# scalable-arch/CAL_22-MPC

Measured on AMD Instinct MI355X. Metric: 64B blocks/s (whole node) + achieved HBM GB/s fraction; ratio bit-exact vs CPU, higher is better.
Workload: dtype u8; 1 GPU; 268435456 random_u32 64 B blocks per GPU, VPC probe config (6 modules, all predictors); algorithm=VPC, line_size=64, blocks_per_gpu=268435456

## Files before the change

cal_22-mpc_amd/csrc/mpc_vpc_lane.hip:

```cpp
#include "mpc_kernel_common.h"
#include "mpc_ring.h"

#ifndef MPC_JIT_BM
#define MPC_JIT_BM 0
#endif
#ifndef MPC_JIT_ANYROOT
#define MPC_JIT_ANYROOT 0
#endif
#ifndef MPC_JIT_PLANES
#define MPC_JIT_PLANES 0
#endif
#ifndef MPC_JIT_GATHER
#define MPC_JIT_GATHER 0
#endif
#ifndef MPC_JIT_WSHIFT
#define MPC_JIT_WSHIFT 0
#endif
#ifndef MPC_ABLATE
#define MPC_ABLATE 0
#endif
namespace {

constexpr int LK_PW = 8;
constexpr int LK_PW2 = 16;
__device__ __host__ constexpr int lk_base(int kind) { return kind & 7; }
__device__ __host__ constexpr int lk_dist(int kind) { return (kind & LK_PW2) ? 2 : ((kind & LK_PW) ? 1 : 0); }

typedef const u32 __attribute__((address_space(4))) *ctab_t;
__device__ __forceinline__ ctab_t lane_tab(const MpcVpcParams &P) { return (ctab_t)(u64)P.tab; }

#if MPC_JIT_ANYROOT || MPC_JIT_GATHER || MPC_JIT_WSHIFT
template <int Q>
__device__ __forceinline__ MpcFastModule lane_fm_const(const MpcVpcParams &P)
{
  MpcFastModule f = P.fm[Q];
#if MPC_JIT_ANYROOT
  constexpr int roots[] = {MPC_JIT_ROOTS};
  f.root = roots[Q];
#endif
#if MPC_JIT_GATHER
  constexpr int gathers[] = {MPC_JIT_GATHERS};
  f.gather = gathers[Q] ? Q + 1 : 0;
#endif
#if MPC_JIT_WSHIFT
  constexpr int wgens[] = {MPC_JIT_WGENS};
  f.wgen = wgens[Q] ? Q + 1 : 0;
#endif
  return f;
}
#define LANE_FM(Q) lane_fm_const<Q>(P)
#else
#define LANE_FM(Q) P.fm[Q]
#endif

template <int W>
struct Lane {
  u32 x[W];
  u32 b0;
  u32 rootb;
  bool gen;
  ctab_t trunc;
};

template <int W>
__device__ __forceinline__ u32 lane_root_bytes(const Lane<W> &c, int root)
{
  const int rw = root >> 2;
  u32 xw = 0;
#pragma unroll
  for (int e = 0; e < (MPC_JIT_ANYROOT ? W : 4); e++) xw = and_or(c.x[e], 0u - (u32)(e == rw), xw);
  return perm(xw, xw, 0x01010101u * (u32)(root & 3));
}
__device__ __forceinline__ u32 lane_onebase_pred(u32 rb, int root, int e)
{
  const u32 here = (e == (root >> 2)) ? (0xffu << (8 * (root & 3))) : 0u;
  return rb & ~here;
}
__device__ __forceinline__ u32 lane_row0_word(u32 msbs, int root, int e)
{
  return (MPC_JIT_ANYROOT && e == 3 && root > 15) ? (msbs & 0x00ffffffu) : msbs;
}
template <int W, int NR>
__device__ __forceinline__ void lane_root_to_front(const Lane<W> &c, int root, u32 (&r)[W])
{
  u32 prev = lane_root_bytes<W>(c, root) & 0xff000000u;
#pragma unroll
  for (int e = 0; e < (MPC_JIT_ANYROOT ? NR : (NR < 4 ? NR : 4)); e++) {
    const u32 sh = alignbyte(r[e], prev, 3);
    const int nb = root + 1 - 4 * e;
    const u32 m = nb >= 4 ? ~0u : (nb <= 0 ? 0u : ((1u << (8 * nb)) - 1u));
    prev = r[e];
    r[e] = mask_sel(m, sh, r[e]);
  }
}

__device__ __forceinline__ u32 msb_of_bsub(u32 a, u32 b) { return ((a | H80) - (b & L7F)) ^ a ^ ~b; }

template <int W>
__device__ __forceinline__ u32 plane_bytes(const u32 (&x)[W], int q, int k)
{
  const u32 s01 = k >= 2 ? 0x07030602u : 0x05010400u;
  const u32 p01 = perm(x[4 * q + 1], x[4 * q], s01), p23 = perm(x[4 * q + 3], x[4 * q + 2], s01);
  return perm(p23, p01, (k & 1) ? 0x07060302u : 0x05040100u);
}

template <int W>
__device__ __forceinline__ u32 shuffled_word(const u32 (&x)[W], int j)
{
  constexpr int NG = W / 4;
  return plane_bytes<W>(x, j % NG, 3 - j / NG);
}

template <int KIND>
__device__ __forceinline__ u32 window_predict(u32 b, u32 c1, u32 c2, const MpcFastModule &fm)
{
  if constexpr (KIND == MPC_FK_DIFF)
    return ((b & L7F) + c1) ^ ((b & H80) ^ c2);
  else if constexpr (KIND == MPC_FK_WEIGHT)
    return (b & c1) | ((b >> fm.rs2) & c2);
  else
    return (((b << fm.ls1) >> fm.rs1) & c1) | (((b << fm.ls2) >> fm.rs2) & c2);
}

#if MPC_JIT_GATHER
template <int W>
__device__ __forceinline__ u32 lane_gather_base(const Lane<W> &c, int q, int e)
{
  constexpr short bases[][4 * W] = {MPC_JIT_BASES};
  u32 half[2];
#pragma unroll
  for (int h = 0; h < 2; h++) {
    const int b0 = bases[q][4 * e + 2 * h], b1 = bases[q][4 * e + 2 * h + 1];
    const u32 w0 = b0 >= 0 ? c.x[b0 >> 2] : 0u, w1 = b1 >= 0 ? c.x[b1 >> 2] : 0u;
    const u32 sel = (b0 >= 0 ? (u32)(b0 & 3) : 0x0cu) | ((b1 >= 0 ? 4u + (u32)(b1 & 3) : 0x0cu) << 8) | 0x0c0c0000u;
    half[h] = perm(w1, w0, sel);
  }
  return perm(half[1], half[0], 0x05040100u);
}
#endif

#if MPC_JIT_WSHIFT
template <int W>
__device__ __forceinline__ u32 lane_weight_general(u32 b, int q, int e)
{
  constexpr signed char sh[][4 * W] = {MPC_JIT_SHIFTS};
  u32 pred = 0;
#pragma unroll
  for (int k = 0; k < 4; k++) {
    const int s = sh[q][4 * e + k];
    if (s == 99) continue;
    const u32 keep = (s >= 0 ? ((0xffu << s) & 0xffu) : (0xffu >> -s)) << (8 * k);
    pred |= (s >= 0 ? (b << s) : (b >> -s)) & keep;
  }
  return pred;
}
#endif

template <int W, int KIND>
__device__ __forceinline__ u32 window_base(const Lane<W> &c, int e, ctab_t t)
{
  constexpr int D = lk_dist(KIND);
  if (D && e >= D) return c.x[e - D];
  return perm(c.x[e], e ? c.x[e - 1] : 0u, t[e]);
}

template <int W, int KIND, bool FULL = true>
__device__ __forceinline__ u32 window_residue(const Lane<W> &c, int e, ctab_t t, const MpcFastModule &fm)
{
#if MPC_JIT_GATHER
  const u32 b = fm.gather ? lane_gather_base<W>(c, fm.gather - 1, e) : window_base<W, KIND>(c, e, t);
#else
  const u32 b = window_base<W, KIND>(c, e, t);
#endif
  constexpr int D = lk_dist(KIND);
  const int k = D == 2 ? (e < 2 ? e : 2 + (e & 1)) : (D == 1 ? (e ? 1 : 0) : e);
  if constexpr (lk_base(KIND) == MPC_FK_WEIGHT) {
    const u32 p7 = ((b >> fm.rs2) & t[2 * W + k]) | (b & t[3 * W + k]);
    const u32 sub = (c.x[e] | H80) - p7;
    const u32 w = c.x[e] ^ (b & t[4 * W + k]);
    return FULL ? (sub ^ (~w & H80)) : (sub ^ ~w);
  } else {
#if MPC_JIT_WSHIFT
    const u32 pred = fm.wgen ? lane_weight_general<W>(b, fm.wgen - 1, e) : window_predict<lk_base(KIND)>(b, t[W + k], t[2 * W + k], fm);
#else
    const u32 pred = window_predict<lk_base(KIND)>(b, t[W + k], t[2 * W + k], fm);
#endif
    return FULL ? bsub(c.x[e], pred) : msb_of_bsub(c.x[e], pred);
  }
}

template <int W, int KIND, int NR = W>
__device__ __forceinline__ void lane_residue(const Lane<W> &c, const MpcFastModule &fm, ctab_t tab,
                                             u32 (&r)[W], u32 &root_r)
{
  root_r = 0;
  if constexpr (lk_base(KIND) == MPC_FK_ONEBASE) {
    if (c.gen && fm.root != 0) {
      const u32 rb = lane_root_bytes<W>(c, fm.root);
#pragma unroll
      for (int e = 0; e < NR; e++) r[e] = bsub(c.x[e], (MPC_JIT_ANYROOT || e < 4) ? lane_onebase_pred(rb, fm.root, e) : rb);
    } else {
      r[0] = bsub(c.x[0], c.rootb & 0xffffff00u);
#pragma unroll
      for (int e = 1; e < NR; e++) r[e] = bsub(c.x[e], c.rootb);
    }
  } else if constexpr (lk_base(KIND) == MPC_FK_CONSEC) {
    u32 in[NR];
#pragma unroll
    for (int j = 0; j < NR; j++) in[j] = shuffled_word<W>(c.x, j);
    r[0] = bsub(c.x[0], in[0] << 8);
#pragma unroll
    for (int e = 1; e < NR; e++) r[e] = bsub(c.x[e], alignbyte(in[e], in[e - 1], 3));
    root_r = (c.b0 - (c.x[0] >> 24)) & 0xffu;
  } else {
    ctab_t t = tab + fm.tab_off;
#pragma unroll
    for (int e = 0; e < NR; e++) r[e] = window_residue<W, KIND>(c, e, t, fm);
  }
}

template <int W, int KIND, int E0, int E1>
__device__ __forceinline__ u32 lane_row0(const Lane<W> &c, const MpcFastModule &fm, ctab_t tab)
{
  u32 m = 0;
  if constexpr (lk_base(KIND) == MPC_FK_ONEBASE) {
    if (c.gen && fm.root != 0) {
      const u32 rb = lane_root_bytes<W>(c, fm.root);
#pragma unroll
      for (int e = E0; e < E1; e++) m |= lane_row0_word(msb_of_bsub(c.x[e], lane_onebase_pred(rb, fm.root, e)), fm.root, e);
      if (MPC_JIT_ANYROOT && E0 == 0 && fm.root > 15) m |= rb;
    } else {
#pragma unroll
      for (int e = E0; e < E1; e++) m |= msb_of_bsub(c.x[e], e ? c.rootb : (c.rootb & 0xffffff00u));
    }
  } else if constexpr (lk_base(KIND) == MPC_FK_CONSEC) {
#pragma unroll
    for (int e = E0; e < E1; e++) {
      const u32 in_e = shuffled_word<W>(c.x, e);
      m |= msb_of_bsub(c.x[e], e ? alignbyte(in_e, shuffled_word<W>(c.x, e - 1), 3) : (in_e << 8));
    }
  } else {
    ctab_t t = tab + fm.tab_off;
#pragma unroll
    for (int e = E0; e < E1; e++) m |= lane_row0_word(window_residue<W, KIND, false>(c, e, t, fm), c.gen ? fm.root : 0, e);
    if (MPC_JIT_ANYROOT && c.gen && E0 == 0 && fm.root > 15) m |= lane_root_bytes<W>(c, fm.root);
  }
  return m & H80;
}

template <int W>
__device__ __forceinline__ u32 lane_leading_zero_rows(const u32 (&r)[W], ctab_t scan_mask = nullptr, u32 plane_mask = ~0u)
{
  constexpr int NG = W / 4;
  u32 S[NG], G = 0;
  if (scan_mask) {
#pragma unroll
    for (int j = 0; j < NG; j++) {
      S[j] = (r[4 * j] & scan_mask[4 * j]) | (r[4 * j + 1] & scan_mask[4 * j + 1]) | (r[4 * j + 2] & scan_mask[4 * j + 2]) |
             (r[4 * j + 3] & scan_mask[4 * j + 3]);
      G |= S[j];
    }
  } else {
#pragma unroll
    for (int j = 0; j < NG; j++) {
      S[j] = r[4 * j] | r[4 * j + 1] | r[4 * j + 2] | r[4 * j + 3];
      G |= S[j];
    }
  }
  const u32 gf = fold8(G) & plane_mask;
  const u32 p = (u32)__clz((int)gf) - 24u;
  const u32 B = H80 >> (p & 7u);
  u32 j_star = NG - 1;
#pragma unroll
  for (int j = NG - 2; j >= 0; j--) j_star = (S[j] & B) ? (u32)j : j_star;
  return (plane_mask == ~0u ? G : gf) ? NG * p + j_star : 2u * W;
}

template <int W>
struct LaneBest {
  u32 r[W];
  u32 z;
  int q;
  u32 root_r;
  u32 cx;
  u32 pm;
  u32 encb;
};

#ifndef MPC_DEFER_MAX
#define MPC_DEFER_MAX 8
#endif

#ifndef MPC_PAIR_PROBE
#define MPC_PAIR_PROBE 64
#endif
constexpr u32 kPairProbe = MPC_PAIR_PROBE;

__host__ __device__ static inline size_t lane_stats_smem(int K, int bins)
{
  return 16 * (size_t)((2 * K * 8 + 15) / 16) + 16 * (size_t)(((K * bins + 2) * 4 + 15) / 16);
}

template <int W, int KIND>
__device__ __forceinline__ u32 lane_row0_bm(const Lane<W> &c, const MpcFastModule &fm, ctab_t tab)
{
  u32 r[W], root_r;
  lane_residue<W, KIND, 1>(c, fm, tab, r, root_r);
  return r[0] & (c.trunc ? (c.trunc[0] & 0xffffu) : 0xffffu);
}

template <int W, int NPT, int Q>
__device__ __forceinline__ u32 lane_row0_min(const Lane<W> &, const MpcVpcParams &) { return ~0u; }

template <int W, int NPT, int Q, int KIND, int... REST>
__device__ __forceinline__ u32 lane_row0_min(const Lane<W> &c, const MpcVpcParams &P)
{
  if constexpr (Q + 1 == NPT) {
    return ~0u;
  } else {
    const u32 m = MPC_JIT_BM ? lane_row0_bm<W, KIND>(c, LANE_FM(Q), lane_tab(P)) : lane_row0<W, KIND, 0, 3>(c, LANE_FM(Q), lane_tab(P));
    return min(m, lane_row0_min<W, NPT, Q + 1, REST...>(c, P));
  }
}

template <int W, int NPT, int Q>
__device__ __forceinline__ u32 lane_prefilters(const Lane<W> &, const MpcVpcParams &, u64 &, u64 &, bool, bool &) { return 0; }

template <int W, int NPT, int Q, int KIND, int... REST>
__device__ __forceinline__ u32 lane_prefilters(const Lane<W> &c, const MpcVpcParams &P, u64 &need_mask, u64 &defer_mask,
                                               bool allow_defer, bool &alt)
{
  if constexpr (Q + 1 == NPT) {
    return 0;
  } else {
    u32 bit = 0;
    if constexpr (!(MPC_ABLATE & 8)) {
      u32 msb = MPC_JIT_BM ? lane_row0_bm<W, KIND>(c, LANE_FM(Q), lane_tab(P)) : lane_row0<W, KIND, 0, 3>(c, LANE_FM(Q), lane_tab(P));
      if ((__ballot(msb != 0) & need_mask) != need_mask) {
        if (!MPC_JIT_BM) msb |= lane_row0<W, KIND, 3, 4>(c, LANE_FM(Q), lane_tab(P));
        const u64 pass = ~__ballot(msb != 0) & need_mask;
        if (pass) {
          if (MPC_DEFER_MAX > 0 && W <= 16 && allow_defer && __popcll(pass) <= MPC_DEFER_MAX) {
            defer_mask |= pass;
            need_mask &= ~pass;
          } else {
            bit = 1u << Q;
            const u64 even = 0x5555555555555555ull;
            if (__popcll(pass) >= 16 && ((pass & even) == 0 || (pass & ~even) == 0) &&
                __popcll(need_mask & ~pass) >= 16)
              alt = true;
          }
        }
      }
    }
    return bit | lane_prefilters<W, NPT, Q + 1, REST...>(c, P, need_mask, defer_mask, allow_defer, alt);
  }
}

template <int W, int NR>
__device__ __forceinline__ u32 lane_leading_zero_rows_bm(const u32 (&r)[W], ctab_t scan_mask, u32 none);

template <int W, int NPT, int Q>
__device__ __forceinline__ void lane_seq(const Lane<W> &, const MpcVpcParams &, u32, LaneBest<W> &, bool) {}

template <int W, int NPT, int Q, int KIND, int... REST>
__device__ __forceinline__ void lane_seq(const Lane<W> &c, const MpcVpcParams &P, u32 keep_bits, LaneBest<W> &best,
                                         bool any_full)
{
  constexpr bool last = Q + 1 == NPT;
  if (last || (keep_bits & (1u << Q))) {
    u32 r[W], root_r;
    lane_residue<W, KIND>(c, LANE_FM(Q), lane_tab(P), r, root_r);
    if (c.gen && LANE_FM(Q).root != 0) lane_root_to_front<W, W>(c, LANE_FM(Q).root, r);
    const u32 pm_q = MPC_JIT_PLANES ? LANE_FM(Q).plane_mask : (c.gen ? P.plane_mask : ~0u);
    const u32 z = MPC_JIT_BM ? lane_leading_zero_rows_bm<W, W>(r, c.gen ? c.trunc : nullptr, 2u * W)
                             : lane_leading_zero_rows<W>(r, c.gen ? c.trunc : nullptr, pm_q);
    if (!any_full) {
      best.z = z;
      best.q = Q;
      best.root_r = root_r;
      best.cx = (u32)LANE_FM(Q).cx;
      best.pm = pm_q;
      best.encb = (u32)P.enc_bits[P.start + Q + 1];
#pragma unroll
      for (int e = 0; e < W; e++) best.r[e] = r[e];
    } else {
      const u32 m = best.z <= z ? ~0u : 0u;
      best.z = mask_sel(m, z, best.z);
      best.q = (int)mask_sel(m, (u32)Q, (u32)best.q);
      best.root_r = mask_sel(m, root_r, best.root_r);
      best.cx = mask_sel(m, (u32)LANE_FM(Q).cx, best.cx);
      if (MPC_JIT_PLANES) best.pm = mask_sel(m, pm_q, best.pm);
      best.encb = mask_sel(m, (u32)P.enc_bits[P.start + Q + 1], best.encb);
#pragma unroll
      for (int e = 0; e < W; e++) best.r[e] = mask_sel(m, r[e], best.r[e]);
    }
    any_full = true;
  }
  if constexpr (!last) lane_seq<W, NPT, Q + 1, REST...>(c, P, keep_bits, best, any_full);
}

template <int W, int NPT, int Q>
__device__ __forceinline__ void lane_last(const Lane<W> &, const MpcVpcParams &, LaneBest<W> &) {}

template <int W, int NPT, int Q, int KIND, int... REST>
__device__ __forceinline__ void lane_last(const Lane<W> &c, const MpcVpcParams &P, LaneBest<W> &best)
{
  if constexpr (Q + 1 == NPT) {
    lane_residue<W, KIND>(c, LANE_FM(Q), lane_tab(P), best.r, best.root_r);
    if (c.gen && LANE_FM(Q).root != 0) lane_root_to_front<W, W>(c, LANE_FM(Q).root, best.r);
    best.q = Q;
    best.cx = (u32)LANE_FM(Q).cx;
    best.pm = MPC_JIT_PLANES ? LANE_FM(Q).plane_mask : ~0u;
    best.encb = (u32)P.enc_bits[P.start + Q + 1];
  } else {
    lane_last<W, NPT, Q + 1, REST...>(c, P, best);
  }
}


template <int W, int NR>
__device__ __forceinline__ u32 lane_leading_zero_rows_bm(const u32 (&r)[W], ctab_t scan_mask, u32 none)
{
  u32 fe = NR, fw = 0;
#pragma unroll
  for (int e = NR - 1; e >= 0; e--) {
    const u32 v = scan_mask ? (r[e] & scan_mask[e]) : r[e];
    fe = v ? (u32)e : fe;
    fw = v ? v : fw;
  }
  const u32 byte = 4u * fe + ((u32)__builtin_ctz(fw | 0x80000000u) >> 3);
  return fe == (u32)NR ? none : (byte >> 1);
}

template <int W>
__device__ __forceinline__ u32 lane_encode_bm(const u32 (&t)[W])
{
  u32 bits = 0;
  u64 Z = 0;
#pragma unroll
  for (int e = 0; e < W; e++) {
    const u32 hw = perm(t[e], t[e], 0x02030001u);
#pragma unroll
    for (int k = 0; k < 2; k++) {
      const u32 h = k ? (hw >> 16) : (hw & 0xffffu);
      const u32 ones = (u32)__popc(h);
      const bool adj = (h & (h >> 1)) != 0u;
      const bool half_empty = (h & 0xff00u) == 0u || (h & 0x00ffu) == 0u;
      const u32 cost = ones == 1u ? 7u : (ones == 2u && adj) ? 8u : half_empty ? 12u : 17u;
      bits += h ? cost : 0u;
      Z |= (u64)(h == 0u ? 1u : 0u) << (2 * e + k);
    }
  }
  const u64 all = W == 32 ? ~0ull : ((1ull << (2 * (W & 31))) - 1ull);
  const u64 starts = Z & ~(Z << 1);
  const u64 longer = starts & (Z >> 1) & all;
  return bits + 4u * (u32)__popcll(starts) + 3u * (u32)__popcll(longer);
}

template <int W>
__device__ __forceinline__ u32 lane_word_at(const u32 (&x)[W], int idx)
{
  u32 w = 0;
#pragma unroll
  for (int e = 0; e < W; e++) w = and_or(x[e], 0u - (u32)(e == idx), w);
  return w;
}

template <int W, int NR>
__device__ __forceinline__ void lane_residue_rt(const Lane<W> &c, const MpcVpcParams &P, const MpcFastModule &fm, u32 (&r)[W],
                                                u32 &root_r)
{
  switch (fm.kind) {
  case MPC_FK_ONEBASE:
    if (fm.root == 0) {
      lane_residue<W, MPC_FK_ONEBASE, NR>(c, fm, lane_tab(P), r, root_r);
    } else {
      const int rw = fm.root >> 2, rk = fm.root & 3;
      const u32 xw = lane_word_at<W>(c.x, rw);
      const u32 rb = ((xw >> (8 * rk)) & 0xffu) * 0x01010101u;
      const u32 here = 0xffu << (8 * rk);
#pragma unroll
      for (int e = 0; e < NR; e++) r[e] = bsub(c.x[e], e == rw ? (rb & ~here) : rb);
      root_r = 0;
    }
    break;
  case MPC_FK_CONSEC: lane_residue<W, MPC_FK_CONSEC, NR>(c, fm, lane_tab(P), r, root_r); break;
  case MPC_FK_DIFF:
    if (fm.prev_word == 2) lane_residue<W, MPC_FK_DIFF | LK_PW2, NR>(c, fm, lane_tab(P), r, root_r);
    else if (fm.prev_word == 1) lane_residue<W, MPC_FK_DIFF | LK_PW, NR>(c, fm, lane_tab(P), r, root_r);
    else lane_residue<W, MPC_FK_DIFF, NR>(c, fm, lane_tab(P), r, root_r);
    break;
  case MPC_FK_WEIGHT:
    if (fm.prev_word == 2) lane_residue<W, MPC_FK_WEIGHT | LK_PW2, NR>(c, fm, lane_tab(P), r, root_r);
    else if (fm.prev_word == 1) lane_residue<W, MPC_FK_WEIGHT | LK_PW, NR>(c, fm, lane_tab(P), r, root_r);
    else lane_residue<W, MPC_FK_WEIGHT, NR>(c, fm, lane_tab(P), r, root_r);
    break;
// ... 209 lines not shown
      u32 Z;
      bits += encode_rows(&t[4 * j], Z);
      ZP |= (u64)Z << (8 * j);
    }
  }
  constexpr u64 all = NG == 8 ? ~0ull : ((1ull << (8 * (NG & 7))) - 1ull);
  const u64 prevP = ((ZP << 8) & all) | (ZP >> (8 * (NG - 1) + 1));
  const u64 nextP = (ZP >> 8) | ((ZP & 0x7full) << (8 * (NG - 1) + 1));
  const u64 starts = ZP & ~prevP;
  return bits + 4u * (u32)__popcll(starts) + 3u * (u32)__popcll(starts & nextP);
}

struct LaneRun {
  u32 key;
  u32 cnt;
  u32 acc_r, acc_r2;
  bool enc_hot;
};

__device__ __forceinline__ void lane_run_flush(const LaneRun &rs, const WgStats &st, int K, int bins)
{
  if (rs.cnt) {
    const int k = (int)(rs.key >> 16);
    atomicAdd(&st.hist[k * bins + (int)(rs.key & 0xffffu)], rs.cnt);
    if (rs.acc_r | rs.acc_r2) {
      atomicAdd(&st.sums[k], (u64)rs.acc_r);
      atomicAdd(&st.sums[K + k], (u64)rs.acc_r2);
    }
  }
}

struct LaneEnv {
  WgStats st;
  int K, bins;
  u32 enc_zero, enc_same, enc_unc;
  u32 n_lines, lane;
  u64 first_line;
  uint16_t *sizes_out;
  int8_t *sel_out;
  u32 *defer_q;
  u32 defer_cap;
};

template <int W>
__device__ __forceinline__ void byte_sums(const u32 (&w)[W], u32 &sum, u32 &sum2)
{
  u32 a0 = 0, a1 = 0, q0 = 0, q1 = 0;
#pragma unroll
  for (int e = 0; e < W; e += 2) {
    a0 = sum_bytes(w[e], a0);
    q0 = sum_sq_bytes(w[e], q0);
    a1 = sum_bytes(w[e + 1], a1);
    q1 = sum_sq_bytes(w[e + 1], q1);
  }
  sum = a0 + a1;
  sum2 = q0 + q1;
}

__device__ __forceinline__ void lane_run_add(LaneRun &rs, u32 key, u32 sum_r, u32 sum_r2, const LaneEnv &E)
{
  if (key != rs.key) {
    lane_run_flush(rs, E.st, E.K, E.bins);
    rs.key = key;
    rs.cnt = 0;
    rs.acc_r = 0;
    rs.acc_r2 = 0;
  }
  rs.cnt++;
  rs.acc_r += sum_r;
  rs.acc_r2 += sum_r2;
}

template <int W, bool OUT, bool GEN, bool FULL, bool DRAIN, int... KINDS>
__device__ __forceinline__ void lane_step(const uint4 (&v)[W / 4], u32 line0, u32 loff, u32 dline, bool dvalid,
                                          const MpcVpcParams &P, const LaneEnv &E, LaneRun &rs, u32 &qn, bool &alt)
{
  constexpr int L = 4 * W;
  constexpr int NQ = W / 4;
  constexpr int NPT = sizeof...(KINDS);
  constexpr u32 uncomp = 8u * L;
  const u32 line = DRAIN ? dline : line0 + loff;
  const bool valid = DRAIN ? dvalid : (FULL ? true : (line < E.n_lines));
  const u64 valid_mask = (FULL && !DRAIN) ? ~0ull : __ballot(valid);
  bool deferred = false;
  Lane<W> c;
  c.gen = GEN;
#pragma unroll
  for (int i = 0; i < NQ; i++) {
    c.x[4 * i] = v[i].x; c.x[4 * i + 1] = v[i].y; c.x[4 * i + 2] = v[i].z; c.x[4 * i + 3] = v[i].w;
  }

  bool is_rep = false, is_zero = false;
  if (__ballot(valid && c.x[1] == c.x[0])) {
    u32 diff = 0;
#pragma unroll
    for (int e = 1; e < W; e++) diff |= c.x[e] ^ c.x[0];
    is_rep = diff == 0;
    is_zero = (diff | c.x[0]) == 0;
  }
  bool need = valid && !(is_zero || (P.has_aws && is_rep));
  u64 need_mask = __ballot(need);

  int chosen = is_zero ? 0 : 1;
  u32 size = is_zero ? E.enc_zero : E.enc_same;
  u32 sum_r = 0, sum_r2 = 0;

  ctab_t scan_mask = ((NPT == 0 || (GEN && P.plane_mask == ~0u)) && P.trunc_off >= 0) ? lane_tab(P) + P.trunc_off : nullptr;
  c.trunc = GEN ? scan_mask : nullptr;
  if (need_mask) {
    c.b0 = c.x[0] & 0xffu;
    c.rootb = perm(c.x[0], c.x[0], 0u);
    LaneBest<W> best;
    if constexpr (NPT > 0) {
      u64 defer_mask = 0;
      const bool allow_defer = !DRAIN && E.defer_cap != 0u && qn + (u32)((NPT - 1) * MPC_DEFER_MAX) <= E.defer_cap;
      u32 keep_bits = 0;
      if ((__ballot(lane_row0_min<W, NPT, 0, KINDS...>(c, P) != 0u) & need_mask) != need_mask)
        keep_bits = lane_prefilters<W, NPT, 0, KINDS...>(c, P, need_mask, defer_mask, allow_defer, alt);
      if (!DRAIN && defer_mask) {
        deferred = (defer_mask >> E.lane) & 1ull;
        const u32 rank = __builtin_amdgcn_mbcnt_hi((u32)(defer_mask >> 32), __builtin_amdgcn_mbcnt_lo((u32)defer_mask, 0u));
        if (deferred) E.defer_q[qn + rank] = line;
        qn += (u32)__popcll(defer_mask);
        need = need && !deferred;
      }
      if (keep_bits == 0) lane_last<W, NPT, 0, KINDS...>(c, P, best);
      else lane_seq<W, NPT, 0, KINDS...>(c, P, keep_bits, best, false);
    } else {
      lane_seq_runtime<W>(c, P, best, scan_mask, need_mask);
    }
    const bool no_pred = NPT == 0 && P.n_pred == 0;
    const u32 unc_size = (no_pred ? 0u : uncomp) + E.enc_unc;

    u32 t[W];
    const u64 cx_mask = __ballot(best.cx != 0);
    if ((cx_mask & need_mask) == need_mask) {
#pragma unroll
      for (int e = 0; e < W; e++) t[e] = best.r[e] ^ ((best.r[e] >> 1) & (e == 0 ? 0x7f7f7f00u : L7F));
    } else {
      const u32 cx7 = best.cx ? L7F : 0u, ncx = best.cx ? 0u : ~0u;
#pragma unroll
      for (int e = 0; e < W; e++) {
        const u32 a = best.r[e] & H80;
        const u32 f = ((best.r[e] >> 1) & cx7) | ((a - (a >> 7)) & ncx);
        t[e] = best.r[e] ^ (e == 0 ? (f & 0xffffff00u) : f);
      }
    }
    if ((NPT == 0 || GEN) && scan_mask) {
#pragma unroll
      for (int e = 0; e < W; e++) t[e] &= scan_mask[e];
    }
    if (MPC_JIT_PLANES && NPT > 0) {
#pragma unroll
      for (int e = 0; e < W; e++) t[e] &= best.pm;
    }
    if (GEN && P.plane_mask != ~0u) {
#pragma unroll
      for (int e = 0; e < W; e++) t[e] &= P.plane_mask;
    }
    bool open = need;
    const bool byte_major = (NPT == 0 && P.byte_major) || (MPC_JIT_BM && NPT > 0);
    if (!rs.enc_hot && !byte_major) open = need && !lane_certified<W>(t);
    if (MPC_JIT_BM && NPT > 0 && !rs.enc_hot) open = need && !lane_certified_bm<W>(t);
    if constexpr (MPC_ABLATE & 16) {
      if (__ballot(open)) E.st.hist[0] = 1u;
      open = false;
    }
    u32 enc = uncomp;
    if (__ballot(open)) {
      if (byte_major) enc = lane_encode_bm<W>(t);
      else enc = lane_encode<W>(t);
    }
    const bool keep = open && enc < uncomp && !no_pred;
    const u64 keep_mask = __ballot(keep);
    rs.enc_hot = keep_mask != 0;

    if (keep_mask == 0 && need_mask == valid_mask) {
      if constexpr (MPC_ABLATE & 4) { sum_r = c.x[3]; sum_r2 = c.x[5]; }
      else byte_sums<W>(c.x, sum_r, sum_r2);
      if (valid) lane_run_add(rs, unc_size, sum_r, sum_r2, E);
      if constexpr (OUT) {
        if (valid) {
          const u64 at = E.first_line + line;
          if (E.sizes_out) E.sizes_out[at] = (uint16_t)unc_size;
          if (E.sel_out) E.sel_out[at] = (int8_t)-1;
        }
      }
      return;
    }
    if (keep_mask == need_mask) {
      const u32 w0 = mask_sel(0xffu, best.root_r, best.r[0]);
      u32 a0 = sum_bytes(w0, 0u), q0 = sum_sq_bytes(w0, 0u), a1 = 0, q1 = 0;
#pragma unroll
      for (int e = 1; e < W; e += 2) {
        a1 = sum_bytes(best.r[e], a1);
        q1 = sum_sq_bytes(best.r[e], q1);
        if (e + 1 < W) {
          a0 = sum_bytes(best.r[e + 1], a0);
          q0 = sum_sq_bytes(best.r[e + 1], q0);
        }
      }
      sum_r = a0 + a1;
      sum_r2 = q0 + q1;
    } else {
      u32 w[W];
      const u32 km = keep ? ~0u : 0u;
#pragma unroll
      for (int e = 0; e < W; e++) w[e] = mask_sel(km, best.r[e], c.x[e]);
      w[0] = mask_sel(km & 0xffu, best.root_r, w[0]);
      byte_sums<W>(w, sum_r, sum_r2);
    }
    sum_r = need ? sum_r : 0u;
    sum_r2 = need ? sum_r2 : 0u;
    if (need) {
      chosen = keep ? P.start + best.q : -1;
      size = keep ? enc + best.encb : unc_size;
    }
  }

  u32 key = ((u32)(chosen + 1) << 16) | size;
  if (!DRAIN) key = deferred ? ((u32)E.K << 16) : key;
  if (valid) lane_run_add(rs, key, sum_r, sum_r2, E);

  if constexpr (OUT) {
    if (valid && !deferred) {
      const u64 at = E.first_line + line;
      if (E.sizes_out) E.sizes_out[at] = (uint16_t)size;
      if (E.sel_out) E.sel_out[at] = (int8_t)chosen;
    }
  }
}

template <int NQ>
__device__ __forceinline__ void lane_fetch(uint4 (&v)[NQ], const uint4 *__restrict__ lines, u32 line, u32 n_lines)
{
  const uint4 *src = lines + (u64)min(line, n_lines - 1u) * NQ;
#pragma unroll
  for (int i = 0; i < NQ; i++) v[i] = src[i];
}

#ifndef MPC_LANE_WAVES
#define MPC_LANE_WAVES 16
#endif
#ifndef MPC_LANE_WAVES_128
#define MPC_LANE_WAVES_128 8
#endif
#ifndef MPC_LANE_WAVES_32
#define MPC_LANE_WAVES_32 16
#endif
__host__ __device__ constexpr int lane_wpb_of(int L) { return L <= 32 ? MPC_LANE_WAVES_32 : (L <= 64 ? MPC_LANE_WAVES : MPC_LANE_WAVES_128); }
template <int W, int NPT>
__host__ __device__ constexpr int lane_wpb() { return NPT == 0 ? 4 : lane_wpb_of(4 * W); }

struct LaneLds {
  u32 stages;
  u32 cap;
  size_t bytes;
};
__host__ __device__ static inline size_t lane_ring_off(size_t stats_and_queues) { return (stats_and_queues + 1023u) & ~(size_t)1023u; }

static LaneLds lane_lds_plan(const MpcVpcParams *P, int wpb, bool wants_queue)
{
  const size_t stats = lane_stats_smem(P->M + 1, P->hist_bins), SB = 64u * (size_t)P->L, lds = 160u << 10;
  const u32 caps[5] = {wants_queue ? 256u : 0u, wants_queue ? 192u : 0u, wants_queue ? 160u : 0u, wants_queue ? 96u : 0u, 0u};
  for (u32 cap : caps) {
    const size_t bytes = lane_ring_off(stats + (size_t)wpb * cap * sizeof(u32)) + (size_t)wpb * 2u * SB;
    if (bytes <= lds) return LaneLds{2, cap, bytes};
  }
  return LaneLds{0, 0, 0};
}

#ifndef MPC_LB_WAVES
#define MPC_LB_WAVES 4
#endif
#ifndef MPC_LB_WAVES_RT
#define MPC_LB_WAVES_RT 3
#endif
#ifndef MPC_LB_WAVES_128
#define MPC_LB_WAVES_128 2
#endif
template <int W, bool OUT, bool GEN, int... KINDS>
__device__ __forceinline__ void vpc_lane_body(unsigned char *smem, const uint4 *__restrict__ lines, u32 n_lines, u64 first_line,
                                              const MpcVpcParams &P, uint16_t *__restrict__ sizes_out, int8_t *__restrict__ sel_out,
                                              u64 *gstats, u32 ring_cfg)
{
  constexpr int NQ = W / 4;
  constexpr u32 WPB = lane_wpb<W, sizeof...(KINDS)>();
  LaneEnv E;
  E.K = P.M + 1;
  E.bins = P.hist_bins;
  E.st.sums = reinterpret_cast<u64 *>(smem);
  E.st.hist = reinterpret_cast<u32 *>(smem + 16 * ((2 * E.K * 8 + 15) / 16));
  if (threadIdx.x == 0) E.st.hist[E.K * E.bins + 1] = 0;
  stats_init(E.st, E.K, E.bins, threadIdx.x, 64 * (int)WPB);
  E.defer_cap = ring_cfg >> 8;
  E.defer_q = reinterpret_cast<u32 *>(smem + lane_stats_smem(E.K, E.bins)) + (threadIdx.x >> 6) * E.defer_cap;
  E.enc_zero = (u32)P.enc_bits[1];
  E.enc_same = 32u + (u32)P.enc_bits[2];
  E.enc_unc = (u32)P.enc_bits[0];
  E.n_lines = n_lines;
  E.lane = threadIdx.x & 63;
  E.first_line = first_line;
  E.sizes_out = sizes_out;
  E.sel_out = sel_out;

  LaneRun rs = {0xffffffffu, 0, 0, 0, false};
  u32 iter = 0;
  const u32 wave = __builtin_amdgcn_readfirstlane(threadIdx.x >> 6);
  u64 *routes = gstats + (2 * E.K + E.K * E.bins);
  (void)routes;
  bool alt = false;
  uint4 va[NQ];
  u32 qn = 0;
  if constexpr (sizeof...(KINDS) == 0) {
    uint4 vb[NQ];
    const u32 stride = gridDim.x * WPB * 64u;
    u32 line0 = (blockIdx.x * WPB + wave) * 64u;
    if (line0 < n_lines) lane_fetch<NQ>(va, lines, line0 + E.lane, n_lines);
    while (line0 < n_lines) {
      lane_fetch<NQ>(vb, lines, line0 + stride + E.lane, n_lines);
      lane_step<W, OUT, false, false, false>(va, line0, E.lane, 0u, true, P, E, rs, qn, alt);
      line0 += stride;
#pragma unroll
      for (int i = 0; i < NQ; i++) va[i] = vb[i];
      if ((++iter & 255u) == 0) {
        lane_run_flush(rs, E.st, E.K, E.bins);
        rs.cnt = 0;
        rs.acc_r = 0;
        rs.acc_r2 = 0;
      }
    }
  } else {
    constexpr u32 SB = 64u * 4u * W;
    constexpr u32 kNone = 0xffffffffu;
    const u32 defer_high = E.defer_cap >= 64u ? E.defer_cap - 64u : 0u;
    const u32 ring_lds = (u32)lane_ring_off(lane_stats_smem(E.K, E.bins) + WPB * E.defer_cap * sizeof(u32)) + wave * (2u * SB);
    u32 lane_off[NQ];
#pragma unroll
    for (int j = 0; j < NQ; j++) lane_off[j] = ring_src_off<NQ>(j, E.lane);
    const u32 rd0 = (ring_lds + 16u * NQ * E.lane) | (16u * ring_swz<NQ>(E.lane));
    const u32 n_blocks = n_lines >> 7;
    const u32 per_wg = uni((n_blocks + gridDim.x - 1u) / gridDim.x);
    const u32 b_begin = blockIdx.x * per_wg;
    const u32 b_end = b_begin + per_wg < n_blocks ? b_begin + per_wg : n_blocks;
    u32 *ticket = E.st.hist + E.K * E.bins + 1;
    auto claim = [&]() -> u32 {
      u32 t = 0;
      if (E.lane == 0) t = atomicAdd(ticket, 1u);
      const u32 blk = b_begin + uni(t);
      return uni((b_begin < n_blocks && blk < b_end) ? blk : kNone);
    };
    auto request = [&](u32 blk, u32 h) { ring_request<NQ>(lane_off, lines + (u64)(2u * blk + h) * (64u * NQ), ring_lds + h * SB); };
    u32 cb = claim();
    if (cb != kNone) {
      request(cb, 0u);
      request(cb, 1u);
    }
    bool paired = false;
    u32 pair_left = 0;
    bool tail_done = false;
    for (;;) {
      while (cb != kNone && qn <= defer_high) {
        cb = uni(cb);
        qn = uni(qn);
        iter = uni(iter);
        const bool pair_now = uni(paired);
        const u32 nb = claim();
        for (u32 h = 0; h < 2u; h = uni(h + 1u)) {
          u32 a0;
          if (pair_now) {
            ring_wait_vm<0>();
            const u32 bl = 2u * E.lane + h;
            a0 = (ring_lds + 16u * NQ * bl) | (16u * ring_swz<NQ>(bl & 63u));
          } else {
            if (uni(h == 0u || nb != kNone)) ring_wait_vm<NQ>();
            else ring_wait_vm<0>();
            a0 = rd0 + h * SB;
          }
          u32 a[NQ];
#pragma unroll
          for (int j = 0; j < NQ; j++) a[j] = a0 ^ (16u * (u32)j);
          ring_read<NQ>(va, a);
          if constexpr (!(MPC_ABLATE & 32)) {
            if (nb != kNone) {
              if (!pair_now) {
                request(nb, h);
              } else if (h == 1u) {
                request(nb, 0u);
                request(nb, 1u);
              }
            }
          }
          __builtin_amdgcn_sched_barrier(0);
          lane_step<W, OUT, GEN, true, false, KINDS...>(va, pair_now ? cb * 128u + h : cb * 128u + h * 64u, pair_now ? 2u * E.lane : E.lane,
                                                   0u, true, P, E, rs, qn, alt);
          if ((++iter & 255u) == 0) {
            lane_run_flush(rs, E.st, E.K, E.bins);
            rs.cnt = 0;
            rs.acc_r = 0;
            rs.acc_r2 = 0;
          }
        }
        alt = uni(alt);
        paired = uni(paired);
        pair_left = uni(pair_left);
        if (MPC_TESTING && E.lane == 0) route_add(routes, pair_now ? MPC_RT_VPC_PAIRED_BLOCKS : MPC_RT_VPC_PLAIN_BLOCKS, 1u);
        if (paired) {
          if (--pair_left == 0u) {
            paired = false;
            if (MPC_TESTING && E.lane == 0) route_add(routes, MPC_RT_VPC_TO_PLAIN, 1u);
          }
        } else if (alt) {
          paired = true;
          pair_left = kPairProbe;
          if (MPC_TESTING && E.lane == 0) route_add(routes, MPC_RT_VPC_TO_PAIRED, 1u);
        }
        alt = false;
        cb = nb;
      }
      const bool tail_mine = !tail_done && cb == kNone && blockIdx.x == gridDim.x - 1u && wave == 0u;
      u32 tail_l0 = n_blocks * 128u;
      for (;;) {
        u32 dline;
        bool dvalid;
        if (qn > 0u) {
          const u32 take = qn < 64u ? qn : 64u;
          qn -= take;
          if (MPC_TESTING && E.lane == 0) {
            route_add(routes, MPC_RT_VPC_DRAINS, 1u);
            route_add(routes, MPC_RT_VPC_DEFERRED, take);
          }
          dvalid = E.lane < take;
          dline = dvalid ? E.defer_q[qn + E.lane] : 0u;
        } else if (tail_mine && tail_l0 < n_lines) {
          dline = tail_l0 + E.lane;
          dvalid = dline < n_lines;
          tail_l0 += 64u;
          if (MPC_TESTING && E.lane == 0) route_add(routes, MPC_RT_VPC_TAIL_GROUPS, 1u);
        } else {
          break;
        }
        lane_fetch<NQ>(va, lines, dline, n_lines);
        lane_step<W, OUT, GEN, false, true, KINDS...>(va, 0u, 0u, dline, dvalid, P, E, rs, qn, alt);
      }
      if (tail_mine) tail_done = true;
      if (cb == kNone && (tail_done || blockIdx.x != gridDim.x - 1u || wave != 0u)) break;
    }
  }
  lane_run_flush(rs, E.st, E.K, E.bins);
  stats_flush(E.st, E.K, E.bins, gstats, (int)(E.lane + 64u * wave), 64 * (int)WPB);
}

#define MPC_LANE_BOUNDS(W, NPT)                                                                                     \
  __launch_bounds__((64 * lane_wpb<W, NPT>()),                                                                      \
                    (W <= 16 ? (NPT > 0 ? (W == 8 && MPC_LANE_WAVES_32 == 10 ? 5 : MPC_LB_WAVES) : MPC_LB_WAVES_RT) : MPC_LB_WAVES_128))
template <int W, bool OUT, int... KINDS>
__global__ void MPC_LANE_BOUNDS(W, (sizeof...(KINDS)))
vpc_lane_kernel(const uint4 *__restrict__ lines, u32 n_lines, u64 first_line, MpcVpcParams P,
                uint16_t *__restrict__ sizes_out, int8_t *__restrict__ sel_out, u64 *gstats, u32 ring_cfg)
{
  extern __shared__ __attribute__((aligned(16))) unsigned char smem[];
  vpc_lane_body<W, OUT, false, KINDS...>(smem, lines, n_lines, first_line, P, sizes_out, sel_out, gstats, ring_cfg);
}
template <int W, bool OUT, int... KINDS>
__global__ void MPC_LANE_BOUNDS(W, (sizeof...(KINDS)))
vpc_lane_gen_kernel(const uint4 *__restrict__ lines, u32 n_lines, u64 first_line, MpcVpcParams P,
                    uint16_t *__restrict__ sizes_out, int8_t *__restrict__ sel_out, u64 *gstats, u32 ring_cfg)
{
  extern __shared__ __attribute__((aligned(16))) unsigned char smem[];
  vpc_lane_body<W, OUT, true, KINDS...>(smem, lines, n_lines, first_line, P, sizes_out, sel_out, gstats, ring_cfg);
}

#ifndef MPC_LANE_JIT
#define OB MPC_FK_ONEBASE
#define CS MPC_FK_CONSEC
#define DF MPC_FK_DIFF
#define WT MPC_FK_WEIGHT

template <int... KINDS>
bool lane_seq_matches(const MpcVpcParams *P)
{
  constexpr int n = sizeof...(KINDS);
  const int kinds[n > 0 ? n : 1] = {KINDS...};
  if (P->n_pred != n || n == 0 || P->runtime_only) return false;
  for (int q = 0; q < n; q++) {
    const MpcFastModule &f = P->fm[q];
    if (f.kind != lk_base(kinds[q])) return false;
    if (lk_dist(kinds[q]) ? f.prev_word != lk_dist(kinds[q]) : f.prev_word == 2) return false;
  }
  return true;
}

template <int... KINDS>
hipError_t lane_launch(const uint4 *l, u32 n_lines, u64 first_line, const MpcVpcParams *P, uint16_t *d_sizes,
                       int8_t *d_sel, u64 *d_stats, int grid, hipStream_t stream)
{
#define MPC_LAUNCH_K(KERNEL, WV, OUTV)                                                                               \
  {                                                                                                                \
    if (smem > (64u << 10))                                                                                        \
      (void)hipFuncSetAttribute(reinterpret_cast<const void *>(&KERNEL<WV, OUTV, KINDS...>),                       \
                                hipFuncAttributeMaxDynamicSharedMemorySize, (int)smem);                            \
    hipLaunchKernelGGL((KERNEL<WV, OUTV, KINDS...>), dim3(wgrid), dim3(64 * wpb), smem, stream, l, n_lines,         \
                       first_line, *P, d_sizes, d_sel, d_stats, ring_cfg);                                         \
  }
#define MPC_LAUNCH(WV)                                                                                              \
  {                                                                                                                \
    constexpr int wpb = lane_wpb<WV, sizeof...(KINDS)>();                                                          \
    size_t smem;                                                                                                   \
    u32 ring_cfg = 0;                                                                                              \
    int wgrid;                                                                                                     \
    if (sizeof...(KINDS) == 0) {                                                                                   \
      smem = lane_stats_smem(P->M + 1, P->hist_bins);                                                              \
      wgrid = grid;                                                                                                \
    } else {                                                                                                       \
      const LaneLds plan = lane_lds_plan(P, wpb, WV <= 16);                                                        \
      if (plan.stages == 0) return hipErrorInvalidConfiguration;              \
      smem = plan.bytes;                                                                                           \
      ring_cfg = plan.stages | (plan.cap << 8);                                                                    \
           \
                 \
      const u64 want = (n_lines / 64u + (u64)wpb - 1u) / (u64)wpb;                                                 \
      const u64 cap = (u64)grid / (wpb == 16 ? 16u : 8u);        \
      wgrid = (int)(want < cap ? want : cap);                                                                      \
      if (wgrid < 1) wgrid = 1;                                                                                    \
    }                                                                                                              \
// ... 177 lines not shown
```

Before: 96.22 billion blocks/s.

## Convert lane_step to wave masks, add bitop3 residues, fast-path uniform run keys

Replaces per-lane booleans in lane_step with wave-wide ballot masks and inverse-ballot lane bits, which cuts repeated ballots and divergent control flow. When only the last predictor runs, it uses compile-time cx, encb and root_r values. Weight and diff residue computations are fused into bitop3/xor3 ternary-logic ops, with a new non-full diff path. A uniform fast path skips lane_run_add when every lane's key matches the current run, and an explicit vmcnt wait is added before drain steps. Together these touch many parts of the kernel, which raises the risk of subtle correctness or register-pressure changes.

```diff
diff --git a/cal_22-mpc_amd/csrc/mpc_vpc_lane.hip b/cal_22-mpc_amd/csrc/mpc_vpc_lane.hip
--- a/cal_22-mpc_amd/csrc/mpc_vpc_lane.hip
+++ b/cal_22-mpc_amd/csrc/mpc_vpc_lane.hip
@@ -15,6 +15,9 @@
 #endif
 #ifndef MPC_JIT_WSHIFT
 #define MPC_JIT_WSHIFT 0
+#endif
+#ifndef MPC_DRAIN_WAIT
+#define MPC_DRAIN_WAIT 1
 #endif
 #ifndef MPC_ABLATE
 #define MPC_ABLATE 0
@@ -177,8 +180,15 @@
   if constexpr (lk_base(KIND) == MPC_FK_WEIGHT) {
     const u32 p7 = ((b >> fm.rs2) & t[2 * W + k]) | (b & t[3 * W + k]);
     const u32 sub = (c.x[e] | H80) - p7;
-    const u32 w = c.x[e] ^ (b & t[4 * W + k]);
-    return FULL ? (sub ^ (~w & H80)) : (sub ^ ~w);
+    const u32 w = bitop3<(BO_A ^ (BO_B & BO_C))>(c.x[e], b, t[4 * W + k]);
+    return FULL ? bitop3<(BO_A ^ (BO_B & ~BO_C)) & 0xFFu>(sub, H80, w) : bitop3<(BO_A ^ ~BO_B) & 0xFFu>(sub, w, w);
+  } else if constexpr (lk_base(KIND) == MPC_FK_DIFF && !FULL) {
+#if MPC_JIT_WSHIFT
+    if (fm.wgen) return msb_of_bsub(c.x[e], lane_weight_general<W>(b, fm.wgen - 1, e));
+#endif
+    const u32 p7 = (b & L7F) + t[W + k];
+    const u32 sub = (c.x[e] | H80) - (p7 & L7F);
+    return bitop3<(BO_A ^ BO_B ^ ~BO_C) & 0xFFu>(xor3(sub, c.x[e], p7), b, t[2 * W + k]);
   } else {
 #if MPC_JIT_WSHIFT
     const u32 pred = fm.wgen ? lane_weight_general<W>(b, fm.wgen - 1, e) : window_predict<lk_base(KIND)>(b, t[W + k], t[2 * W + k], fm);
@@ -275,6 +285,8 @@
   for (int j = NG - 2; j >= 0; j--) j_star = (S[j] & B) ? (u32)j : j_star;
   return (plane_mask == ~0u ? G : gf) ? NG * p + j_star : 2u * W;
 }
+
+__device__ __forceinline__ bool lane_bit(u64 mask) { return __builtin_amdgcn_inverse_ballot_w64(mask); }
 
 template <int W>
 struct LaneBest {
@@ -400,6 +412,14 @@
   if constexpr (!last) lane_seq<W, NPT, Q + 1, REST...>(c, P, keep_bits, best, any_full);
 }
 
+template <int... KINDS>
+__device__ __host__ constexpr bool lane_last_has_root_r()
+{
+  constexpr int n = sizeof...(KINDS);
+  constexpr int kinds[n > 0 ? n : 1] = {KINDS...};
+  return n > 0 && lk_base(kinds[n > 0 ? n - 1 : 0]) == MPC_FK_CONSEC;
+}
+
 template <int W, int NPT, int Q>
 __device__ __forceinline__ void lane_last(const Lane<W> &, const MpcVpcParams &, LaneBest<W> &) {}
 
@@ -407,12 +427,10 @@
 __device__ __forceinline__ void lane_last(const Lane<W> &c, const MpcVpcParams &P, LaneBest<W> &best)
 {
   if constexpr (Q + 1 == NPT) {
-    lane_residue<W, KIND>(c, LANE_FM(Q), lane_tab(P), best.r, best.root_r);
+    u32 zero_root_r;
+    lane_residue<W, KIND>(c, LANE_FM(Q), lane_tab(P), best.r, lk_base(KIND) == MPC_FK_CONSEC ? best.root_r : zero_root_r);
     if (c.gen && LANE_FM(Q).root != 0) lane_root_to_front<W, W>(c, LANE_FM(Q).root, best.r);
-    best.q = Q;
-    best.cx = (u32)LANE_FM(Q).cx;
     best.pm = MPC_JIT_PLANES ? LANE_FM(Q).plane_mask : ~0u;
-    best.encb = (u32)P.enc_bits[P.start + Q + 1];
   } else {
     lane_last<W, NPT, Q + 1, REST...>(c, P, best);
   }
@@ -788,7 +806,6 @@
   const u32 line = DRAIN ? dline : line0 + loff;
   const bool valid = DRAIN ? dvalid : (FULL ? true : (line < E.n_lines));
   const u64 valid_mask = (FULL && !DRAIN) ? ~0ull : __ballot(valid);
-  bool deferred = false;
   Lane<W> c;
   c.gen = GEN;
 #pragma unroll
@@ -796,20 +813,22 @@
     c.x[4 * i] = v[i].x; c.x[4 * i + 1] = v[i].y; c.x[4 * i + 2] = v[i].z; c.x[4 * i + 3] = v[i].w;
   }
 
-  bool is_rep = false, is_zero = false;
+  u64 zero_mask = 0, rep_mask = 0;
   if (__ballot(valid && c.x[1] == c.x[0])) {
     u32 diff = 0;
 #pragma unroll
     for (int e = 1; e < W; e++) diff |= c.x[e] ^ c.x[0];
-    is_rep = diff == 0;
-    is_zero = (diff | c.x[0]) == 0;
-  }
-  bool need = valid && !(is_zero || (P.has_aws && is_rep));
-  u64 need_mask = __ballot(need);
-
-  int chosen = is_zero ? 0 : 1;
-  u32 size = is_zero ? E.enc_zero : E.enc_same;
+    rep_mask = __ballot(valid && diff == 0);
+    zero_mask = __ballot(valid && (diff | c.x[0]) == 0);
+  }
+  u64 need_mask = valid_mask & ~(zero_mask | (P.has_aws ? rep_mask : 0ull));
+  u64 defer_mask = 0;
+
   u32 sum_r = 0, sum_r2 = 0;
+  int n_chosen;
+  u32 n_size;
+  bool all_unc = false;
+  u32 key = 0;
 
   ctab_t scan_mask = ((NPT == 0 || (GEN && P.plane_mask == ~0u)) && P.trunc_off >= 0) ? lane_tab(P) + P.trunc_off : nullptr;
   c.trunc = GEN ? scan_mask : nullptr;
@@ -817,34 +836,38 @@
     c.b0 = c.x[0] & 0xffu;
     c.rootb = perm(c.x[0], c.x[0], 0u);
     LaneBest<W> best;
+    u32 keep_bits = 0;
     if constexpr (NPT > 0) {
-      u64 defer_mask = 0;
       const bool allow_defer = !DRAIN && E.defer_cap != 0u && qn + (u32)((NPT - 1) * MPC_DEFER_MAX) <= E.defer_cap;
-      u32 keep_bits = 0;
       if ((__ballot(lane_row0_min<W, NPT, 0, KINDS...>(c, P) != 0u) & need_mask) != need_mask)
         keep_bits = lane_prefilters<W, NPT, 0, KINDS...>(c, P, need_mask, defer_mask, allow_defer, alt);
       if (!DRAIN && defer_mask) {
-        deferred = (defer_mask >> E.lane) & 1ull;
         const u32 rank = __builtin_amdgcn_mbcnt_hi((u32)(defer_mask >> 32), __builtin_amdgcn_mbcnt_lo((u32)defer_mask, 0u));
-        if (deferred) E.defer_q[qn + rank] = line;
+        if (lane_bit(defer_mask)) E.defer_q[qn + rank] = line;
         qn += (u32)__popcll(defer_mask);
-        need = need && !deferred;
       }
       if (keep_bits == 0) lane_last<W, NPT, 0, KINDS...>(c, P, best);
       else lane_seq<W, NPT, 0, KINDS...>(c, P, keep_bits, best, false);
     } else {
       lane_seq_runtime<W>(c, P, best, scan_mask, need_mask);
     }
+    u32 kb = keep_bits;
+    asm volatile("" : "+s"(kb));
+    const bool last_only = NPT > 0 && kb == 0;
+    u32 last_cx = 0;
+    if constexpr (NPT > 0) last_cx = (u32)LANE_FM(NPT - 1).cx;
     const bool no_pred = NPT == 0 && P.n_pred == 0;
     const u32 unc_size = (no_pred ? 0u : uncomp) + E.enc_unc;
 
     u32 t[W];
-    const u64 cx_mask = __ballot(best.cx != 0);
+    const u32 best_root_r = (last_only && !lane_last_has_root_r<KINDS...>()) ? 0u : best.root_r;
+    const u64 cx_mask = last_only ? (last_cx ? ~0ull : 0ull) : __ballot(best.cx != 0);
     if ((cx_mask & need_mask) == need_mask) {
 #pragma unroll
       for (int e = 0; e < W; e++) t[e] = best.r[e] ^ ((best.r[e] >> 1) & (e == 0 ? 0x7f7f7f00u : L7F));
     } else {
-      const u32 cx7 = best.cx ? L7F : 0u, ncx = best.cx ? 0u : ~0u;
+      const u32 bcx = last_only ? last_cx : best.cx;
+      const u32 cx7 = bcx ? L7F : 0u, ncx = bcx ? 0u : ~0u;
 #pragma unroll
       for (int e = 0; e < W; e++) {
         const u32 a = best.r[e] & H80;
@@ -864,27 +887,28 @@
 #pragma unroll
       for (int e = 0; e < W; e++) t[e] &= P.plane_mask;
     }
-    bool open = need;
+    u64 open_mask = need_mask;
     const bool byte_major = (NPT == 0 && P.byte_major) || (MPC_JIT_BM && NPT > 0);
-    if (!rs.enc_hot && !byte_major) open = need && !lane_certified<W>(t);
-    if (MPC_JIT_BM && NPT > 0 && !rs.enc_hot) open = need && !lane_certified_bm<W>(t);
+    if (!rs.enc_hot && !byte_major) open_mask &= ~__ballot(lane_certified<W>(t));
+    if (MPC_JIT_BM && NPT > 0 && !rs.enc_hot) open_mask &= ~__ballot(lane_certified_bm<W>(t));
     if constexpr (MPC_ABLATE & 16) {
-      if (__ballot(open)) E.st.hist[0] = 1u;
-      open = false;
+      if (open_mask) E.st.hist[0] = 1u;
+      open_mask = 0;
     }
     u32 enc = uncomp;
-    if (__ballot(open)) {
+    u64 keep_mask = 0;
+    if (open_mask) {
       if (byte_major) enc = lane_encode_bm<W>(t);
       else enc = lane_encode<W>(t);
-    }
-    const bool keep = open && enc < uncomp && !no_pred;
-    const u64 keep_mask = __ballot(keep);
+      if (!no_pred) keep_mask = __ballot(enc < uncomp) & open_mask;
+    }
     rs.enc_hot = keep_mask != 0;
 
     if (keep_mask == 0 && need_mask == valid_mask) {
       if constexpr (MPC_ABLATE & 4) { sum_r = c.x[3]; sum_r2 = c.x[5]; }
       else byte_sums<W>(c.x, sum_r, sum_r2);
-      if (valid) lane_run_add(rs, unc_size, sum_r, sum_r2, E);
+      all_unc = true;
+      key = unc_size;
       if constexpr (OUT) {
         if (valid) {
           const u64 at = E.first_line + line;
@@ -892,50 +916,71 @@
           if (E.sel_out) E.sel_out[at] = (int8_t)-1;
         }
       }
-      return;
-    }
-    if (keep_mask == need_mask) {
-      const u32 w0 = mask_sel(0xffu, best.root_r, best.r[0]);
-      u32 a0 = sum_bytes(w0, 0u), q0 = sum_sq_bytes(w0, 0u), a1 = 0, q1 = 0;
-#pragma unroll
-      for (int e = 1; e < W; e += 2) {
-        a1 = sum_bytes(best.r[e], a1);
-        q1 = sum_sq_bytes(best.r[e], q1);
-        if (e + 1 < W) {
-          a0 = sum_bytes(best.r[e + 1], a0);
-          q0 = sum_sq_bytes(best.r[e + 1], q0);
+    } else {
+      const bool keep = lane_bit(keep_mask);
+      if (keep_mask == need_mask) {
+        const u32 w0 = mask_sel(0xffu, best_root_r, best.r[0]);
+        u32 a0 = sum_bytes(w0, 0u), q0 = sum_sq_bytes(w0, 0u), a1 = 0, q1 = 0;
+#pragma unroll
+        for (int e = 1; e < W; e += 2) {
+          a1 = sum_bytes(best.r[e], a1);
+          q1 = sum_sq_bytes(best.r[e], q1);
+          if (e + 1 < W) {
+            a0 = sum_bytes(best.r[e + 1], a0);
+            q0 = sum_sq_bytes(best.r[e + 1], q0);
+          }
         }
+        sum_r = a0 + a1;
+        sum_r2 = q0 + q1;
+      } else {
+        u32 w[W];
+        const u32 km = keep ? ~0u : 0u;
+#pragma unroll
+        for (int e = 0; e < W; e++) w[e] = mask_sel(km, best.r[e], c.x[e]);
+        w[0] = mask_sel(km & 0xffu, best_root_r, w[0]);
+        byte_sums<W>(w, sum_r, sum_r2);
       }
-      sum_r = a0 + a1;
-      sum_r2 = q0 + q1;
-    } else {
-      u32 w[W];
-      const u32 km = keep ? ~0u : 0u;
-#pragma unroll
-      for (int e = 0; e < W; e++) w[e] = mask_sel(km, best.r[e], c.x[e]);
-      w[0] = mask_sel(km & 0xffu, best.root_r, w[0]);
-      byte_sums<W>(w, sum_r, sum_r2);
-    }
-    sum_r = need ? sum_r : 0u;
-    sum_r2 = need ? sum_r2 : 0u;
-    if (need) {
-      chosen = keep ? P.start + best.q : -1;
-      size = keep ? enc + best.encb : unc_size;
-    }
-  }
-
-  u32 key = ((u32)(chosen + 1) << 16) | size;
-  if (!DRAIN) key = deferred ? ((u32)E.K << 16) : key;
-  if (valid) lane_run_add(rs, key, sum_r, sum_r2, E);
-
-  if constexpr (OUT) {
-    if (valid && !deferred) {
-      const u64 at = E.first_line + line;
-      if (E.sizes_out) E.sizes_out[at] = (uint16_t)size;
-      if (E.sel_out) E.sel_out[at] = (int8_t)chosen;
-    }
-  }
-}
+      const bool need = lane_bit(need_mask);
+      sum_r = need ? sum_r : 0u;
+      sum_r2 = need ? sum_r2 : 0u;
+      if (keep_mask) {
+        u32 last_encb = 0;
+        if constexpr (NPT > 0) last_encb = (u32)P.enc_bits[P.start + NPT];
+        n_chosen = keep ? P.start + (last_only ? NPT - 1 : best.q) : -1;
+        n_size = keep ? enc + (last_only ? last_encb : best.encb) : unc_size;
+      } else {
+        n_chosen = -1;
+        n_size = unc_size;
+      }
+    }
+  }
+
+  if (!all_unc) {
+    const bool is_zero = lane_bit(zero_mask), need = lane_bit(need_mask), deferred = !DRAIN && lane_bit(defer_mask);
+    const int chosen = need ? n_chosen : (is_zero ? 0 : 1);
+    const u32 size = need ? n_size : (is_zero ? E.enc_zero : E.enc_same);
+    key = ((u32)(chosen + 1) << 16) | size;
+    if (!DRAIN) key = deferred ? ((u32)E.K << 16) : key;
+
+    if constexpr (OUT) {
+      if (valid && !deferred) {
+        const u64 at = E.first_line + line;
+        if (E.sizes_out) E.sizes_out[at] = (uint16_t)size;
+        if (E.sel_out) E.sel_out[at] = (int8_t)chosen;
+      }
+    }
+  }
+
+  if (FULL && !DRAIN && __ballot(key != rs.key) == 0) {
+    rs.cnt++;
+    rs.acc_r += sum_r;
+    rs.acc_r2 += sum_r2;
+  } else if (valid) {
+    lane_run_add(rs, key, sum_r, sum_r2, E);
+  }
+}
+
+constexpr int kWaitVm0 = (7 << 4) | (15 << 8);
 
 template <int NQ>
 __device__ __forceinline__ void lane_fetch(uint4 (&v)[NQ], const uint4 *__restrict__ lines, u32 line, u32 n_lines)
@@ -1062,7 +1107,7 @@
       request(cb, 0u);
       request(cb, 1u);
     }
-    bool paired = false;
+    u32 paired = 0;
     u32 pair_left = 0;
     bool tail_done = false;
     for (;;) {
@@ -1070,7 +1115,7 @@
         cb = uni(cb);
         qn = uni(qn);
         iter = uni(iter);
-        const bool pair_now = uni(paired);
+        const u32 pair_now = uni(paired);
         const u32 nb = claim();
         for (u32 h = 0; h < 2u; h = uni(h + 1u)) {
           u32 a0;
@@ -1079,7 +1124,7 @@
             const u32 bl = 2u * E.lane + h;
             a0 = (ring_lds + 16u * NQ * bl) | (16u * ring_swz<NQ>(bl & 63u));
           } else {
-            if (uni(h == 0u || nb != kNone)) ring_wait_vm<NQ>();
+            if (h == 0u || nb != kNone) ring_wait_vm<NQ>();
             else ring_wait_vm<0>();
             a0 = rd0 + h * SB;
           }
@@ -1113,11 +1158,11 @@
         if (MPC_TESTING && E.lane == 0) route_add(routes, pair_now ? MPC_RT_VPC_PAIRED_BLOCKS : MPC_RT_VPC_PLAIN_BLOCKS, 1u);
         if (paired) {
           if (--pair_left == 0u) {
-            paired = false;
+            paired = 0u;
             if (MPC_TESTING && E.lane == 0) route_add(routes, MPC_RT_VPC_TO_PLAIN, 1u);
           }
         } else if (alt) {
-          paired = true;
+          paired = 1u;
           pair_left = kPairProbe;
           if (MPC_TESTING && E.lane == 0) route_add(routes, MPC_RT_VPC_TO_PAIRED, 1u);
         }
@@ -1147,6 +1192,7 @@
           break;
         }
         lane_fetch<NQ>(va, lines, dline, n_lines);
+        if constexpr (MPC_DRAIN_WAIT) __builtin_amdgcn_s_waitcnt(kWaitVm0);
         lane_step<W, OUT, GEN, false, true, KINDS...>(va, 0u, 0u, dline, dvalid, P, E, rs, qn, alt);
       }
       if (tail_mine) tail_done = true;
```

After: 101.0 billion blocks/s, median of 6. 1.05x the previous value.
